# fusiyuan2010/CSC

Measured on AMD Instinct MI355X. Metric: encode MB/s (10^6 input bytes / wall-clock) on enwik9 stand-in, -m3 -d64m; stream bit-exact vs reference, higher is better.
Workload: dtype u8/u32 (byte + 32-bit integer work; 12-bit probabilities, 64-bit range-coder low)

## Files before the change

### csc_amd/csrc/csc_kernels_dp4.inc

```

constexpr uint32_t kD4Rec = 256;
constexpr uint32_t kD4CandEnt = kD4Rec * 4;
constexpr uint32_t kD4RefEnt = 256;
constexpr uint32_t kD4Ent = kD4CandEnt + kD4RefEnt;
constexpr uint32_t kD4LA = 48;
constexpr uint32_t kD4Waves = 12;
DEV uint32_t d4_role(uint32_t w)
{
    constexpr uint32_t roles[12] = { 0, 6, 7, 1, 8, 5, 4, 2, 8, 8, 9, 3 };
    return w < 12 ? roles[w] : 8u;
}
constexpr uint32_t kD4Requested = 0xFFFFFFFFu;
#ifndef D4_IDLE_MUL
#define D4_IDLE_MUL 1
#endif
constexpr int kD4IdleSleep = 4 * D4_IDLE_MUL;
constexpr uint32_t kD4RefreshAt = 32;
constexpr uint32_t kD4MaxGood = 16;
constexpr uint32_t kD6Ring = 128;
constexpr uint32_t kD6MRing = 64;
constexpr uint32_t kD4MultiMax = 768;

struct Dp4X {
    uint32_t sb_seq, sb_ack, quit, abort;
    uint32_t sb0, pos0, size, gen;
    uint32_t m_pos;
    uint32_t m_ids[2];
    uint32_t ins_head;
    uint32_t cmp_next, cmp_pause, cmp_idle[3], cmp_cur[3];
    uint32_t ev_seq, ev_s, ev_len, ev_ack;
    uint32_t ref_head;
    uint32_t rq_head, rq_tail;
    uint32_t lit_req, lit_from, lit_done;
    uint32_t rid[4];
    uint32_t io_w0, io_gen, io_state0, io_lp_int, io_lit_seq, io_rq_head, io_wnd_lo, io_wnd_hi, io_wnd_size, io_vld, io_good, io_plit_lo, io_plit_hi;
    alignas(16) uint32_t o_kind, o_end, o_a0l, o_a0code, o_a0eid, o_a0slot, o_fin_i0, o_fin_i1, o_lp_int, o_lit_seq, o_rq_head, o_err;
#ifdef CSCMI_TIMERS
    uint32_t stat[8];
    uint32_t wtm[52];
#endif
    uint32_t rq[16][2];
    raw_vec4 cand[kD4Rec];
    uint8_t hflag[kD4Rec];
    uint32_t rec_tag[kD4Rec], rec_hsum[kD4Rec], rec_a0d[kD4Rec], rec_len[kD4Rec][16];
    uint32_t rec_m32[kD4Rec][16];
    raw_vec4 ent[kD4Ent];
    uint32_t fwd[kD4Ent];
    alignas(512) uint16_t litp[4][kD4Rec];
    alignas(16) uint16_t tab[64][32];
    alignas(256) raw_vec4 lab[16];
    alignas(512) uint32_t tent[2][16][8];
    alignas(256) raw_vec4 ver[16];
    uint32_t lab_seq, win_seq;
    alignas(16) uint32_t dump[8];
    alignas(8) uint32_t e_prog[2]; uint32_t e_stop[2];
#ifdef CSCMI_TIMERS
    uint32_t dbgp[64], dbgq[64][8], dbgl[32];
    uint32_t dbg;
    uint32_t tr_win, tr_lo, tr_hi;
#endif
    uint32_t lenp_new[32];
    uint32_t lt_pub, lt_done;
    uint32_t lt_rec[kD6Ring];
    uint32_t mt_pub, mt_done;
    uint32_t mt_rec[kD6MRing][2];
    uint32_t hS[2], h_reset, hand[20];
};
struct EncLds4 { EncLds base; Dp4X x; CoderQ q; };
__shared__ EncLds4 g_lds4;

DEV uint32_t d4_tag(uint32_t gen, uint32_t p) { return ((gen << 13) | p) + 1u; }
DEV Dp4X *d4x(Sc &c) { return reinterpret_cast<Dp4X *>(c.X); }

DEV uint32_t d4_eq4(uint32_t x)
{
    const uint32_t z = ~(((x & 0x7F7F7F7Fu) + 0x7F7F7F7Fu) | x) & 0x80808080u;
    return (((z >> 7) * 0x01020408u) >> 24) & 0xFu;
}
DEV uint32_t d4_eq8(uint64_t x) { return d4_eq4((uint32_t)x) | (d4_eq4((uint32_t)(x >> 32)) << 4); }

DEV bool d4_spin(Sc &c, Dp4X *X, uint32_t &spins, uint32_t site)
{
    __builtin_amdgcn_s_sleep(1);
    if ((++spins & 1023u) == 0 && (spins > (kDpSpinLimit << 2) || lds_vload(&X->abort))) {
        if (!lds_vload(&X->abort)) lds_vstore(&X->abort, 0x40000000u | (site << 16) | (c.wv << 24) | (spins & 0xFFFFu));
        c.error = lds_vload(&X->abort);
        return false;
    }
    return true;
}
template <int LANE> DEV uint32_t d4_wrlane(uint32_t old, uint32_t val)
{
// ... 1745 lines not shown
    if (!d6_tree_record(c, X, 0u | (len << 1), dist, d6_len_slots(len) + sbits + ndir + (extra_bits ? 4u : 0u), q)) return false;
    c.state = (c.state * 4 + 1) & 0x3F;
    c.st_match++;
    return true;
}
DEV bool d6_rep_match(Sc &c, Dp4X *X, uint32_t rep_idx, uint32_t len, D6Cur &q)
{
    const uint32_t s3 = c.state * 3, k = c.lane;
    const uint32_t idx = k < 3 ? P_STATE + s3 + k : P_REPDIST + s3 - 1u + (k == 3 ? 1u : 2u | (rep_idx >> 1));
    const uint32_t bit = k < 3 ? (0x5u >> k) & 1u : (rep_idx >> ((4u - k) & 1u)) & 1u;
    d6_flags(c, 5, idx, bit);
    if (!d6_tree_record(c, X, 1u | (len << 1), 0u, d6_len_slots(len), q)) return false;
    c.state = (c.state * 4 + 3) & 0x3F;
    c.st_match++;
    return true;
}
DEV void d6_rep0len1(Sc &c)
{
    d6_flags(c, 3, P_STATE + c.state * 3 + c.lane, c.lane == 0 ? 1u : 0u);
    c.ctx = 0;
    c.state = (c.state * 4 + 2) & 0x3F;
    c.st_match++;
}
DEV bool d6_encode_nonlit(Sc &c, Dp4X *X, uint32_t ulen, uint32_t udist, D6Cur &q)
{
    EncLds *L = c.L;
    if (udist <= 4) {
        if (ulen == 1 && udist == 1) d6_rep0len1(c);
        else {
            if (!d6_rep_match(c, X, udist - 1, ulen - 2, q)) return false;
            uint32_t d = UNI(L->rep[udist - 1]);
            for (uint32_t k = udist - 1; k > 0; k--) L->rep[k] = UNI(L->rep[k - 1]);
            L->rep[0] = d;
        }
    } else {
        if (!d6_match(c, X, udist - 5, ulen - 2, q)) return false;
        uint32_t r0 = UNI(L->rep[0]), r1 = UNI(L->rep[1]), r2 = UNI(L->rep[2]);
        L->rep[3] = r2; L->rep[2] = r1; L->rep[1] = r0; L->rep[0] = udist - 4;
    }
    return true;
}
DEV uint32_t d6_chunk_shape(uint32_t nd, uint32_t ql, bool on)
{
    const uint32_t len = ql & 0xFFFFu;
    const uint32_t kind = nd == 0 ? 0u : nd > 4 ? 1u : (nd == 1 && len == 1) ? 2u : 3u;
    const uint32_t l2 = len - 2u, dist = nd - 5u;
    const uint32_t sbits = l2 == 0 ? 3u : l2 <= 2 ? 4u : 5u;
    const uint32_t slot = dist_slot(dist), extra_bits = slot > 2 ? slot - 2 : 0;
    const uint32_t ndir = extra_bits > 4 ? (extra_bits - 4 > 16 ? 2u : 1u) : 0u;
    const uint32_t nf = kind == 0 ? 1u : kind == 1 ? 2u : kind == 2 ? 3u : 5u;
    const uint32_t tree = kind == 0 ? 8u : kind == 2 ? 0u : d6_len_slots(l2) + (kind == 1 ? sbits + ndir + (extra_bits ? 4u : 0u) : 0u);
    return on ? kind | (nf << 2) | ((nf + tree) << 8) : 0u;
}
DEV void d6_chunk_flag(bool act, uint32_t idx, uint32_t bit, uint32_t qslot, uint64_t same)
{
    const uint64_t am = __ballot(act);
    if (am == 0) return;
    const uint32_t lane = threadIdx.x & 63u;
    same &= am;
    const uint64_t below = same & ((1ull << lane) - 1ull), above = (same >> lane) >> 1;
    const uint32_t rank = (uint32_t)__builtin_popcountll(below);
    const uint32_t prev = below ? 63u - (uint32_t)__builtin_clzll(below) : lane;
    uint32_t pold = 0;
    if (act) pold = g_lds4.base.P[idx];
    uint32_t pnew = p_update(bit, pold);
    for (uint32_t d = 1; __ballot(act && rank >= d) != 0; d++) {
        const uint32_t v = (uint32_t)__builtin_amdgcn_ds_bpermute((int)(prev * 4u), (int)pnew);
        if (act && rank == d) { pold = v; pnew = p_update(bit, pold); }
    }
    if (act && above == 0) g_lds4.base.P[idx] = pnew;
    if (act) g_lds4.q.e[qslot & (kCoderQ - 1)] = 0x80000000u | (bit << 12) | pold;
}
__device__ __noinline__ uint32_t d6_chunk_lanes(uint32_t nd, uint32_t ql, uint32_t shape, uint32_t qpos, uint32_t n_, uint32_t state0_, uint32_t ctx0_, uint32_t lt_head_, uint32_t mt_head_)
{
    Dp4X *X = &g_lds4.x;
    const uint32_t lane = threadIdx.x & 63u;
    const uint32_t n = UNI(n_), state0 = UNI(state0_), ctx0 = UNI(ctx0_), lt_head = UNI(lt_head_), mt_head = UNI(mt_head_);
    const bool on = lane < n;
    const uint32_t kind = shape & 3u, nf = (shape >> 2) & 7u;
    const uint32_t len = ql & 0xFFFFu, last = ql >> 16;
    const uint64_t b0 = __ballot(on && (kind & 1u)), b1 = __ballot(on && (kind & 2u));
    const uint64_t h0 = (b0 << 3) | ((state0 & 1u) << 2) | (((state0 >> 2) & 1u) << 1) | ((state0 >> 4) & 1u);
    const uint64_t h1 = (b1 << 3) | (((state0 >> 1) & 1u) << 2) | (((state0 >> 3) & 1u) << 1) | ((state0 >> 5) & 1u);
    const uint32_t a = (uint32_t)(lane >= 3 ? b0 >> (lane - 3u) : h0 >> lane) & 7u, b = (uint32_t)(lane >= 3 ? b1 >> (lane - 3u) : h1 >> lane) & 7u;
    const uint32_t state = ((a >> 2) & 1u) | (((b >> 2) & 1u) << 1) | (((a >> 1) & 1u) << 2) | (((b >> 1) & 1u) << 3) | ((a & 1u) << 4) | ((b & 1u) << 5);
    const uint32_t before = (uint32_t)__shfl_up((int)last, 1);
    const uint32_t ctx = lane == 0 ? ctx0 : before;
    const bool is_lit = on && kind == 0, has_tree = on && (kind & 1u);
    const uint64_t lm = __ballot(is_lit), tm = __ballot(has_tree);
    if (is_lit) {
        const uint32_t r = __builtin_amdgcn_mbcnt_hi((uint32_t)(lm >> 32), __builtin_amdgcn_mbcnt_lo((uint32_t)lm, 0u));
        *(lds_vu32 *)&X->lt_rec[(lt_head + r) & (kD6Ring - 1)] = ctx | (last << 8) | (qpos << 16);
    }
    if (lm) lds_vstore(&X->lt_pub, lt_head + (uint32_t)__builtin_popcountll(lm));
    if (has_tree) {
        const uint32_t r = __builtin_amdgcn_mbcnt_hi((uint32_t)(tm >> 32), __builtin_amdgcn_mbcnt_lo((uint32_t)tm, 0u));
        *(lds_vu32 *)&X->mt_rec[(mt_head + r) & (kD6MRing - 1)][0] = (kind == 3 ? 1u : 0u) | ((len - 2u) << 1) | ((qpos + nf) << 16);
        *(lds_vu32 *)&X->mt_rec[(mt_head + r) & (kD6MRing - 1)][1] = kind == 1 ? nd - 5u : 0u;
    }
    if (tm) lds_vstore(&X->mt_pub, mt_head + (uint32_t)__builtin_popcountll(tm));
    uint64_t same = 0;
    for (uint64_t rem = __ballot(on); rem;) {
        const uint32_t sv = rdlane(state, (uint32_t)__builtin_ctzll(rem));
        const uint64_t mm = __ballot(on && state == sv);
        same = state == sv ? mm : same;
        rem &= ~mm;
    }
    const uint32_t s3 = state * 3u, rep_hi = ((nd - 1u) >> 1) & 1u;
    const bool is_rep = on && kind == 3;
    d6_chunk_flag(on, P_STATE + s3, kind != 0 ? 1u : 0u, qpos, same);
    d6_chunk_flag(on && kind != 0, P_STATE + s3 + 1u, kind == 1 ? 1u : 0u, qpos + 1u, same);
    d6_chunk_flag(on && kind >= 2, P_STATE + s3 + 2u, kind == 3 ? 1u : 0u, qpos + 2u, same);
    d6_chunk_flag(is_rep, P_REPDIST + s3, rep_hi, qpos + 3u, same);
    const uint64_t hi = __ballot(is_rep && rep_hi);
    d6_chunk_flag(is_rep, P_REPDIST + s3 + 1u + rep_hi, (nd - 1u) & 1u, qpos + 4u, same & (rep_hi ? hi : ~hi));
    return rdlane(((state * 4u + kind) & 0x3Fu) | (last << 8), n - 1u);
}
struct D6Rec {
    uint32_t len;
    uint32_t k0[3], nb[3], x[3], base[3];
    uint32_t n, n_head;
    uint32_t ndir, dir0, dir1;
};
DEV D6Rec d6_rec(uint32_t w0, uint32_t dist)
{
    D6Rec r;
    const uint32_t len = (w0 >> 1) & 0xFFu;
    r.len = len;
    r.k0[0] = len < 8 ? 1u : 2u; r.nb[0] = len < 16 ? 3u : 7u; r.x[0] = len < 8 ? len : len < 16 ? len - 8u : len - 16u;
    r.base[0] = len < 8 ? (uint32_t)P_LEN_X1 : len < 16 ? (uint32_t)P_LEN_X2 : (uint32_t)P_LEN_X3;
    uint32_t n = r.k0[0] + r.nb[0];
    const bool match = (w0 & 1u) == 0;
    const uint32_t sbits = len == 0 ? 3u : len <= 2 ? 4u : 5u;
    const uint32_t pdist_pos = len == 0 ? 0u : len <= 2 ? 16u * (len - 1u) + 8u : 32u * (umin(len, 6u) - 3u) + 8u + 16u * 2u;
    const uint32_t slot = dist_slot(dist), extra_bits = match && slot > 2 ? slot - 2u : 0u;
    r.k0[1] = n; r.nb[1] = match ? sbits : 0u; r.x[1] = slot; r.base[1] = P_DIST + pdist_pos;
    n += r.nb[1];
    r.n_head = n;
    const uint32_t extra_len = dist - (1u << (extra_bits & 31u)) - 1u;
    r.k0[2] = n; r.nb[2] = extra_bits ? 4u : 0u; r.x[2] = __brev(extra_len & 0x0Fu) >> 28; r.base[2] = P_DIST_EXTRA + (extra_bits - 1u) * 16u;
    n += r.nb[2];
    r.n = n;
    const uint32_t v = extra_len >> 4, l = extra_bits - 4u;
    r.ndir = extra_bits > 4 ? (l > 16 ? 2u : 1u) : 0u;
    r.dir0 = l <= 16 ? (l << 16) | (v & 0xFFFFu) : ((l - 16u) << 16) | ((v >> 16) & 0xFFFFu);
    r.dir1 = (16u << 16) | (v & 0xFFFFu);
    return r;
}
DEV void d6_rec_cell(const D6Rec &r, uint32_t k, uint32_t &idx, uint32_t &bit)
{
    idx = P_LEN_SLOT; bit = r.len >= 8 ? 1u : 0u;
    if (k == 1 && r.len >= 8) { idx = P_LEN_SLOT + 1; bit = r.len >= 16 ? 1u : 0u; }
#pragma unroll
    for (uint32_t s = 0; s < 3; s++) {
        const uint32_t l = k - r.k0[s];
        if (l < r.nb[s]) { idx = r.base[s] + ((1u << l) | (r.x[s] >> ((r.nb[s] - l) & 31u))); bit = (r.x[s] >> ((r.nb[s] - 1u - l) & 31u)) & 1u; }
    }
}
DEV uint32_t d6_rec_lane(const D6Rec &r, uint32_t idx)
{
    uint32_t k = 0xFFu;
    if (idx == P_LEN_SLOT) k = 0;
    if (idx == P_LEN_SLOT + 1 && r.len >= 8) k = 1;
#pragma unroll
    for (uint32_t s = 0; s < 3; s++) {
        const uint32_t node = idx - r.base[s];
        const uint32_t l = 31u - (uint32_t)__builtin_clz(node | 1u);
        if (node >= 1u && node < (1u << r.nb[s]) && node == ((1u << l) | (r.x[s] >> ((r.nb[s] - l) & 31u)))) k = r.k0[s] + l;
// ... 95 lines not shown
            prev_a = (i >= j && o == cell_a) ? j : prev_a;
            const uint32_t o2 = (uint32_t)__builtin_amdgcn_ds_bpermute((int)((lane + 8u * j) * 4u), (int)cell_a);
            later_a = later_a || (i + j < 8u && o2 == cell_a);
        }
        uint32_t from_a = 0;
        if (n_b) {
#pragma unroll
            for (uint32_t j = 7; j >= 1; j--) {
                const uint32_t o = (uint32_t)__builtin_amdgcn_ds_bpermute((int)((lane - 8u * j) * 4u), (int)cell_b);
                prev_b = (i >= j && o == cell_b) ? j : prev_b;
                const uint32_t o2 = (uint32_t)__builtin_amdgcn_ds_bpermute((int)((lane + 8u * j) * 4u), (int)cell_b);
                later_b = later_b || (i + j < 8u && o2 == cell_b);
            }
#pragma unroll
            for (uint32_t j = 0; j < 8; j++) {
                const uint32_t r = (i + j) & 7u;
                const uint32_t oa = (uint32_t)__builtin_amdgcn_ds_bpermute((int)((lane + 8u * j) * 4u), (int)cell_a);
                from_a = (oa == cell_b && r + 1u > from_a) ? r + 1u : from_a;
                const uint32_t ob = (uint32_t)__builtin_amdgcn_ds_bpermute((int)((lane + 8u * j) * 4u), (int)cell_b);
                later_a = later_a || ob == cell_a;
            }
        }
        uint32_t pnew_a = p_update(bit_a, pold_a);
        const uint64_t cm_a = __ballot(prev_a != 0);
        if (__builtin_expect(cm_a != 0, 0)) {
            for (uint32_t r = 1; r < n_a; r++) {
                if (((cm_a >> (8u * r)) & 0xFFull) == 0) continue;
                const uint32_t v = (uint32_t)__builtin_amdgcn_ds_bpermute((int)((lane - 8u * prev_a) * 4u), (int)pnew_a);
                if (i == r && prev_a != 0) { pold_a = v; pnew_a = p_update(bit_a, pold_a); }
            }
        }
        if (n_b) {
            if (__ballot(from_a != 0)) {
                const uint32_t v = (uint32_t)__builtin_amdgcn_ds_bpermute((int)(((from_a - 1u) * 8u + k) * 4u), (int)pnew_a);
                pold_b = from_a ? v : pold_b;
            }
            uint32_t pnew_b = p_update(bit_b, pold_b);
            const uint64_t cm_b = __ballot(prev_b != 0);
            if (__builtin_expect(cm_b != 0, 0)) {
                for (uint32_t r = 1; r < n_b; r++) {
                    if (((cm_b >> (8u * r)) & 0xFFull) == 0) continue;
                    const uint32_t v = (uint32_t)__builtin_amdgcn_ds_bpermute((int)((lane - 8u * prev_b) * 4u), (int)pnew_b);
                    if (i == r && prev_b != 0) { pold_b = v; pnew_b = p_update(bit_b, pold_b); }
                }
            }
            if (act_b && !later_b) c.p_lit[cell_b] = pnew_b;
            if (act_b) g_lds4.q.e[((rec_b >> 16) + 1u + k) & (kCoderQ - 1)] = 0x80000000u | (bit_b << 12) | pold_b;
        }
        if (act_a && !later_a) c.p_lit[cell_a] = pnew_a;
        if (act_a) g_lds4.q.e[((rec_a >> 16) + 1u + k) & (kCoderQ - 1)] = 0x80000000u | (bit_a << 12) | pold_a;
        dp_fence();
        done += nlit;
        lds_vstore(&X->lt_done, done);
        pub = lds_vload(&X->lt_pub);
    }
  }
}

DEV void lz_compress_advanced_dp4(Sc &c, uint32_t size)
{
    EncLds *L = c.L;
    Dp4X *X = d4x(c);
    const uint32_t lane = c.lane;
    const uint32_t sb0 = c.wnd_curpos, pos0 = c.pos;
    uint32_t rq_head = lds_vload(&X->rq_head);
    uint32_t ev_seq = lds_vload(&X->ev_seq);
    bool ev_pending = false;
    {
        lds_vstore(&X->sb0, sb0); lds_vstore(&X->pos0, pos0); lds_vstore(&X->size, size);
        lds_vstore(&X->m_pos, 0);
        {
            const uint64_t wa = (uint64_t)(uintptr_t)c.wnd;
            X->io_wnd_lo = (uint32_t)wa; X->io_wnd_hi = (uint32_t)(wa >> 32); X->io_wnd_size = c.wnd_size; X->io_vld = c.vld_rge; X->io_good = c.lz_good_len;
            const uint64_t pa = (uint64_t)(uintptr_t)c.p_lit;
            X->io_plit_lo = (uint32_t)pa; X->io_plit_hi = (uint32_t)(pa >> 32);
        }
        dp_fence();
        const uint32_t seq = lds_vload(&X->sb_seq) + 1;
        lds_vstore(&X->sb_seq, seq);
        uint32_t spins = 0;
        while (lds_vload(&X->sb_ack) != seq) if (!d4_spin(c, X, spins, 5)) return;
        lds_fence();
        uint32_t id0 = 0;
        if (lane == 0) id0 = atomicAdd(&X->ref_head, 4u);
        id0 = UNI(id0);
        if (lane < 4) {
            const uint32_t nid = kD4CandEnt + ((id0 + lane) & (kD4RefEnt - 1));
            raw_vec4 en;
            en.x = L->rep[lane]; en.y = sb0 - 64u; en.z = 0; en.w = 0;
            X->ent[nid] = en;
            X->fwd[nid] = 0;
            X->rid[lane] = nid;
        }
        lds_fence();
        if (!d4_rebase_reps(c, X, sb0, rq_head, true)) return;
    }
    uint32_t gen = lds_vload(&X->gen);
    uint32_t lit_seq = lds_vload(&X->lit_req);
    D6Cur tq;
    tq.lt_head = lds_vload(&X->lt_pub); tq.lt_seen = lds_vload(&X->lt_done); tq.mt_head = lds_vload(&X->mt_pub); tq.mt_seen = lds_vload(&X->mt_done);

    for (uint32_t i = 0; i < size;) {
        if (lds_vload(&X->abort)) { c.error = lds_vload(&X->abort); return; }
        TM_DECL;
        const uint32_t w0 = i;
        lds_vstore(&X->m_pos, i);
        if (ev_pending) {
            uint32_t spins = 0;
            while (lds_vload(&X->ev_ack) != ev_seq) if (!d4_spin(c, X, spins, 6)) return;
            lds_fence();
            gen = lds_vload(&X->gen);
            ev_pending = false;
        }
        TM_ADD(c, 0);
        {
            const uint32_t rs = w0 & (kD4Rec - 1);
            const uint32_t tg = *(lds_vu32 *)&X->rec_tag[rs], hs = *(lds_vu32 *)&X->rec_hsum[rs];
            const uint32_t rid_l = *(lds_vu32 *)&X->rid[lane & 3u];
            const raw_vec4 en = *(lds_vvec4 *)&X->ent[rid_l];
            const uint32_t wpos = sb0 + w0, off = wpos - en.y;
            const uint32_t mlow = (uint32_t)((((uint64_t)en.w << 32) | en.z) >> (off & 63u));
            const uint32_t bad = (off >> 6) | ((((off & 63u) + 1u) >> 6) & mlow) | ((umin(en.x - en.y - 1u, 0x7FFFFFFFu) - off) >> 31) | (((mlow & 3u) + 1u) >> 2);
            if (UNI(tg) == d4_tag(gen, w0) && (UNI(hs) & 0xFFu) == 0 && __ballot(bad != 0) == 0 && w0 + 1u < size && !D5FLAG(30)) {
                if (!d6_room(c, X, 16u, tq)) return;
                if (!d6_literal(c, X, stage_byte(c, sb0 + w0), tq)) return;
                TM_ADD(c, 4);
                c.st_find++;
                i++;
                continue;
            }
        }
        if (!d6_join(c, X, tq, true)) return;
        TM_ADD(c, 5);
        if (__builtin_expect(c.error != 0, 0)) { if (!lds_vload(&X->abort)) lds_vstore(&X->abort, c.error); return; }
        X->io_w0 = w0; X->io_gen = gen; X->io_state0 = c.state; X->io_lp_int = c.lp_rebuild_int; X->io_lit_seq = lit_seq; X->io_rq_head = rq_head;
        lds_fence();
#ifdef CSCMI_TIMERS
        if (D5DBG(32u) && c.lane < 32) X->dbgl[c.lane] = L->len_price[c.lane];
#endif
#ifdef CSCMI_TIMERS
        const bool d5_here = (lds_vload(&X->dbg) >> 8) == 0 || D5DBG(64u) || pos0 + w0 < (lds_vload(&X->dbg) >> 8) * 16u;
#else
        const bool d5_here = true;
#endif
#ifdef CSCMI_TIMERS
        if (kD5Split && !D5DBG(16u) && d5_here) d5_spine();
        else d4_window();
#else
        (void)d5_here;
        d5_spine();
#endif
#ifdef CSCMI_TIMERS
        if (D5DBG(128u) && pos0 + w0 + 1024u >= (lds_vload(&X->dbg) >> 8) * 16u) { for (int q = 0; q < 100; q++) __builtin_amdgcn_s_sleep(127); }
#endif
#ifdef CSCMI_TIMERS
        if (D5DBG(32u) && lds_vload(&X->o_end) < 150u && c.S->stats.trace[62][0] == 0
            && (!D5DBG(64u) || (pos0 + w0 < (lds_vload(&X->dbg) >> 8) * 16u && pos0 + w0 + 16u >= (lds_vload(&X->dbg) >> 8) * 16u))) {
            auto sig = [&]() -> uint32_t {
                uint32_t h = lds_vload(&X->o_kind) * 0x9E3779B1u + lds_vload(&X->o_end);
                h = h * 0x85EBCA6Bu + lds_vload(&X->o_a0l); h = h * 0x85EBCA6Bu + lds_vload(&X->o_a0code); h = h * 0x85EBCA6Bu + lds_vload(&X->o_lp_int);
                if (lds_vload(&X->o_kind) == DP_EXIT_MATCH) { h = h * 0x85EBCA6Bu + lds_vload(&X->o_a0slot); if (lds_vload(&X->o_a0code) > 4) h = h * 0x85EBCA6Bu + UNI(X->ent[lds_vload(&X->o_a0eid)].x); }
                { const uint32_t f0 = lds_vload(&X->o_fin_i0), f1 = lds_vload(&X->o_fin_i1);
                  h = h * 31u + UNI(X->ent[f0 & 0xFFFFu].x); h = h * 31u + UNI(X->ent[f0 >> 16].x); h = h * 31u + UNI(X->ent[f1 & 0xFFFFu].x); h = h * 31u + UNI(X->ent[f1 >> 16].x); }
                for (uint32_t t = lds_vload(&X->o_end); t;) {
                    const uint32_t b = UNI(L->fin2[t * 2u + 1u] & 0xFFFFu), d = UNI(L->fin2[t * 2u]);
                    h = (h ^ (t * 31u + d)) * 0x01000193u;
                    t = b;
                }
                return h;
            };
            auto sig2 = [&]() -> uint32_t {
                uint32_t h = 0;
                for (uint32_t q = 0; q < 32; q++) h = h * 31u + UNI(L->len_price[q]);
                return h;
            };
            auto snap = [&](unsigned long long *T) {
                uint32_t hf = 0, he = 0;
                for (uint32_t q = c.lane; q < kD4Ent; q += 64) { hf += X->fwd[q] * (q * 2u + 1u); const raw_vec4 e = X->ent[q]; he += (e.x * 3u + e.y * 5u + e.z * 7u + e.w * 11u) * (q * 2u + 1u); }
                for (int o = 32; o; o >>= 1) { hf += __shfl_xor(hf, o); he += __shfl_xor(he, o); }
                if (c.lane == 0) {
                    T[0] = hf; T[1] = he; T[2] = lds_vload(&X->ref_head); T[3] = lds_vload(&X->rq_head) | ((unsigned long long)lds_vload(&X->rq_tail) << 32);
                    T[4] = lds_vload(&X->lit_req) | ((unsigned long long)lds_vload(&X->lit_done) << 32); T[5] = lds_vload(&X->m_pos);
                    T[6] = lds_vload(&X->m_ids[0]) | ((unsigned long long)lds_vload(&X->m_ids[1]) << 32); T[7] = lds_vload(&X->gen) | ((unsigned long long)lds_vload(&X->ins_head) << 32);
                    T[8] = lds_vload(&X->o_fin_i0) | ((unsigned long long)lds_vload(&X->o_fin_i1) << 32); T[9] = lds_vload(&X->o_kind) | ((unsigned long long)lds_vload(&X->o_end) << 32);
                    T[10] = lds_vload(&X->o_a0eid) | ((unsigned long long)lds_vload(&X->o_a0slot) << 32); T[11] = pos0 + w0;
// ... 8 lines not shown
            X->io_lit_seq = lds_vload(&X->o_lit_seq);
            if (c.lane < 32) L->len_price[c.lane] = X->dbgl[c.lane];
            lds_fence();
            d4_window();
            const uint32_t s4 = sig();
            if (D5DBG(64u)) snap(c.S->stats.trace[59]);
            const uint32_t t4 = sig2();
            if (t4 != t5 && c.S->stats.trace[62][0] == 0 && c.lane == 0) { unsigned long long *T = c.S->stats.trace[62]; T[0] = 2; T[1] = pos0 + w0; T[2] = t5; T[3] = t4; T[4] = lds_vload(&X->io_lp_int); T[5] = lds_vload(&X->o_lp_int); T[6] = lds_vload(&X->o_end); }
            if (s4 != s5 && c.S->stats.trace[62][0] == 0) {
                if (c.lane < 60) { c.S->stats.trace[c.lane][2] = L->fin2[c.lane * 2u]; c.S->stats.trace[c.lane][3] = L->fin2[c.lane * 2u + 1u] & 0xFFFFu; c.S->stats.trace[c.lane][4] = X->dbgp[c.lane]; for (int q = 0; q < 7; q++) c.S->stats.trace[c.lane][5 + q] = X->dbgq[c.lane][q == 6 ? 7 : q]; c.S->stats.trace[c.lane][11] |= (unsigned long long)X->dbgq[c.lane][6] << 32; }
                if (c.lane == 0) {
                    unsigned long long *T = c.S->stats.trace[62];
                    T[0] = 1; T[1] = pos0 + w0; T[2] = k5; T[3] = e5; T[4] = l5; T[5] = a5; T[6] = c5;
                    T[7] = lds_vload(&X->o_kind); T[8] = lds_vload(&X->o_end); T[9] = lds_vload(&X->o_lp_int); T[10] = lds_vload(&X->o_a0l); T[11] = lds_vload(&X->io_lp_int);
                    unsigned long long *U = c.S->stats.trace[63];
                    const uint32_t q0 = lds_vload(&X->o_fin_i0), q1 = lds_vload(&X->o_fin_i1);
                    U[1] = r5a; U[2] = r5b; U[3] = r5c; U[4] = r5d; U[5] = sl5; U[6] = X->ent[q0 & 0xFFFFu].x; U[7] = X->ent[q0 >> 16].x; U[8] = X->ent[q1 & 0xFFFFu].x; U[9] = X->ent[q1 >> 16].x; U[10] = lds_vload(&X->o_a0slot);
                }
            }
        }
#endif
        const raw_vec4 o0 = *(lds_vvec4 *)&X->o_kind, o1 = *(lds_vvec4 *)&X->o_a0eid, o2 = *(lds_vvec4 *)&X->o_lp_int;
        const uint32_t kind = UNI(o0.x), end = UNI(o0.y);
        uint32_t a0l = UNI(o0.z);
        const uint32_t a0code = UNI(o0.w), a0eid = UNI(o1.x), a0slot = UNI(o1.y);
        const uint32_t fin_i0 = UNI(o1.z), fin_i1 = UNI(o1.w);
        c.lp_rebuild_int = UNI(o2.x); lit_seq = UNI(o2.y); rq_head = UNI(o2.z);
        c.st_find += end + (kind == DP_EXIT_LIMIT ? 0u : 1u);
        TM_ADD(c, 1);
#ifdef CSCMI_TIMERS
        if (D5FLAG(29) && c.S->stats.trace[62][0] == 0) {
            const uint32_t thr = lds_vload(&X->tr_win) & 0x1FFFFFFFu;
            if (sb0 + w0 <= thr && thr < sb0 + w0 + end + 1u + (kind == DP_EXIT_MATCH ? a0l : 0u)) {
                if (c.lane < 60) { c.S->stats.trace[c.lane][0] = L->fin2[c.lane * 2u]; c.S->stats.trace[c.lane][1] = L->fin2[c.lane * 2u + 1u]; }
                if (c.lane == 0) {
                    unsigned long long *T = c.S->stats.trace[62];
                    T[0] = 7; T[1] = sb0 + w0; T[2] = kind; T[3] = end; T[4] = a0l; T[5] = a0code; T[6] = a0slot; T[7] = X->ent[fin_i0 & 0xFFFFu].x; T[8] = X->ent[fin_i0 >> 16].x;
                    T[9] = X->ent[fin_i1 & 0xFFFFu].x; T[10] = X->ent[fin_i1 >> 16].x; T[11] = c.state;
                    unsigned long long *U = c.S->stats.trace[63];
                    U[1] = L->rep[0]; U[2] = L->rep[1]; U[3] = L->rep[2]; U[4] = L->rep[3]; U[5] = fin_i0; U[6] = fin_i1; U[7] = X->rid[0] | ((unsigned long long)X->rid[1] << 32); U[8] = X->rid[2] | ((unsigned long long)X->rid[3] << 32);
                    U[9] = X->fwd[X->rid[0]]; U[10] = X->ent[X->rid[0]].y; U[11] = lds_vload(&X->rq_head) | ((unsigned long long)lds_vload(&X->rq_tail) << 32);
                }
            }
        }
#endif
        if (kind == DP_ABORT || UNI(o2.w)) { c.error = lds_vload(&X->abort) | 0x08000000u; return; }
        if (kind == DP_SEEN_EXIT) {
            if (lane < 4) X->rid[lane] = lane == 0 ? fin_i0 & 0xFFFFu : lane == 1 ? fin_i0 >> 16 : lane == 2 ? fin_i1 & 0xFFFFu : fin_i1 >> 16;
            wave_fence();
            if (!d6_room(c, X, 16u, tq)) return;
            if (!d6_literal(c, X, stage_byte(c, sb0 + w0), tq)) return;
            i++;
            TM_ADD(c, 7);
            continue;
        }
        c.wnd_curpos = sb0 + w0 + end;
        if (kind == DP_EXIT_MATCH) {
            if (a0l >= 64u && a0slot >= 4) {
                const uint32_t mp = sb0 + w0 + end, d = a0code - 4u;
                const bool fwd = a0slot == 4 ? (mp > d) : (mp >= d);
                const uint32_t cp = fwd ? mp - d : mp + c.wnd_size - d;
                a0l = wave_prefix_from(c, mp, cp, 64u, umin(size - (w0 + end), c.wnd_size - cp));
            }
            lds_vstore(&X->ev_s, w0 + end); lds_vstore(&X->ev_len, a0l);
            lds_fence();
            ev_seq++;
            lds_vstore(&X->ev_seq, ev_seq);
            ev_pending = true;
        }
        {
            const uint32_t id = lane == 0 ? fin_i0 & 0xFFFFu : lane == 1 ? fin_i0 >> 16 : lane == 2 ? fin_i1 & 0xFFFFu : fin_i1 >> 16;
            if (lane < 4) { X->rid[lane] = id; L->rep[lane] = X->ent[id].x; }
        }
        wave_fence();
        if (kind == DP_EXIT_MATCH) {
            const uint32_t i0 = lds_vload(&X->rid[0]), i1 = lds_vload(&X->rid[1]), i2 = lds_vload(&X->rid[2]), i3 = lds_vload(&X->rid[3]);
            if (a0code > 4) { X->rid[0] = a0eid; X->rid[1] = i0; X->rid[2] = i1; X->rid[3] = i2; }
            else if (a0code == 2) { X->rid[0] = i1; X->rid[1] = i0; }
            else if (a0code == 3) { X->rid[0] = i2; X->rid[1] = i0; X->rid[2] = i1; }
            else if (a0code == 4) { X->rid[0] = i3; X->rid[1] = i0; X->rid[2] = i1; X->rid[3] = i2; }
            wave_fence();
            if (a0l > kD4RefreshAt && w0 + end + a0l < size && !d4_rebase_reps(c, X, sb0 + w0 + end + a0l, rq_head, false)) return;
        }
        TM_ADD(c, 6);
        uint32_t pm_lo = 0, pm_hi = 0;
        for (uint32_t t = end; t;) {
            const uint32_t ch = t >> 6;
            const uint32_t Bv = L->fin2[(ch * 64u + lane) * 2u + 1u] & 0xFFFFu;
            uint64_t m = 0;
            do { m |= 1ull << (t & 63u); t = rdlane(Bv, t & 63u); } while (t && (t >> 6) == ch);
            pm_lo = d4_m0_wrlane(pm_lo, UNI((uint32_t)m), UNI(ch));
            pm_hi = d4_m0_wrlane(pm_hi, UNI((uint32_t)(m >> 32)), UNI(ch));
        }
        TM_ADD(c, 2);
        for (uint32_t ch = 0; ch <= (end >> 6); ch++) {
            const uint64_t m = ((uint64_t)rdlane(pm_hi, ch) << 32) | rdlane(pm_lo, ch);
            if (m == 0) continue;
            const uint32_t n = (uint32_t)__builtin_popcountll(m);
            const uint32_t q = ch * 64u + lane;
            const uint32_t back = L->fin2[q * 2u + 1u] & 0xFFFFu, ndv = L->fin2[q * 2u];
            const uint32_t sidx = w0 + q + 15u;
            const uint32_t lastb = (L->stage[sidx >> 2] >> ((sidx & 3u) * 8u)) & 0xFFu;
            const bool isp = (m >> lane) & 1ull;
            const uint32_t rank = __builtin_amdgcn_mbcnt_hi((uint32_t)(m >> 32), __builtin_amdgcn_mbcnt_lo((uint32_t)m, 0u));
            const uint32_t tgt = (isp ? rank : n + (lane - rank)) * 4u;
            const uint32_t d_nd = (uint32_t)__builtin_amdgcn_ds_permute((int)tgt, (int)ndv);
// ... 3 lines not shown
#pragma unroll
            for (uint32_t b = 0; b < 5; b++) {
                const uint64_t pm = __ballot((shape >> (8u + b)) & 1u);
                qoff += __builtin_amdgcn_mbcnt_hi((uint32_t)(pm >> 32), __builtin_amdgcn_mbcnt_lo((uint32_t)pm, 0u)) << b;
                need += (uint32_t)__builtin_popcountll(pm) << b;
            }
            const uint32_t nl = (uint32_t)__builtin_popcountll(__ballot(lane < n && (shape & 3u) == 0)), nm = (uint32_t)__builtin_popcountll(__ballot(shape & 1u));
            if (!d6_room(c, X, need, tq)) return;
            if (tq.lt_head + nl - tq.lt_seen > kD6Ring - 8u) tq.lt_seen = lds_vload(&X->lt_done);
            if (tq.mt_head + nm - tq.mt_seen > kD6MRing) tq.mt_seen = lds_vload(&X->mt_done);
            const bool at_once = c.q_room >= need && tq.lt_head + nl - tq.lt_seen <= kD6Ring - 8u && tq.mt_head + nm - tq.mt_seen <= kD6MRing;
            TM_ADD(c, 3);
            if (at_once) {
                const uint32_t sc = UNI(d6_chunk_lanes(d_nd, d_ql, shape, c.q_head + qoff, n, c.state, c.ctx, tq.lt_head, tq.mt_head));
                c.state = sc & 0x3Fu; c.ctx = sc >> 8;
                c.q_head += need; c.q_room -= need;
                tq.lt_head += nl; tq.mt_head += nm;
                c.st_lit += nl; c.st_match += n - nl;
                continue;
            }
            for (uint32_t r = 0; r < n; r++) {
                const uint32_t nd = rdlane(d_nd, r), ql = rdlane(d_ql, r);
                const uint32_t len = ql & 0xFFFFu, last = ql >> 16;
                if (nd == 0) {
                    if (!d6_literal(c, X, last, tq)) return;
                    TMF_ADD(c, 4);
                } else if (nd <= 4) {
                    if (len == 1 && nd == 1) d6_rep0len1(c);
                    else if (!d6_rep_match(c, X, nd - 1, len - 2, tq)) return;
                    c.ctx = last;
                    TMF_ADD(c, 7);
                } else {
                    if (!d6_match(c, X, nd - 5, len - 2, tq)) return;
                    c.ctx = last;
                    TMF_ADD(c, 7);
                }
            }
        }
        i += end;
        if (!d6_room(c, X, 256u, tq)) return;
        if (kind == DP_EXIT_LIT) {
            if (!d6_literal(c, X, stage_byte(c, sb0 + i), tq)) return;
            i++;
        } else if (kind == DP_EXIT_MATCH) {
            if (a0l >= 145u) {
                if (!d6_join(c, X, tq)) return;
                lz_encode_nonlit(c, a0l, a0code);
            } else if (!d6_encode_nonlit(c, X, a0l, a0code, tq)) return;
            c.st_slide += a0l - 1;
            i += a0l;
            c.ctx = stage_byte(c, sb0 + i - 1);
        }
        TM_ADD(c, 7);
    }
    if (!d6_join(c, X, tq)) return;
    {
        lds_vstore(&X->m_pos, size);
        uint32_t spins = 0;
        if (ev_pending) { while (lds_vload(&X->ev_ack) != ev_seq) if (!d4_spin(c, X, spins, 9)) return; }
        while (lds_vload(&X->ins_head) < size) if (!d4_spin(c, X, spins, 10)) return;
        if (!d4_quiesce(c, X)) return;
        dp_fence();
    }
    c.pos = pos0 + size;
    c.wnd_curpos = sb0 + size;
}

__device__ __noinline__ void d4_master_nl()
{
    Dp4X *X = &g_lds4.x;
    Sc c;
    const uint64_t sp = ((uint64_t)lds_vload(&X->hS[1]) << 32) | lds_vload(&X->hS[0]);
    const GLOBAL_AS EncState *G = (const GLOBAL_AS EncState *)(uintptr_t)sp;
    c.S = (EncState *)(uintptr_t)sp; c.L = &g_lds4.base; c.X = X; c.Q = &g_lds4.q;
    c.lane = threadIdx.x & 63;
    c.wnd = (gu8 *)uni_gptr(G->wnd); c.wnd_size = UNI(G->wnd_size); c.vld_rge = UNI(G->vld_rge);
    c.ht2 = nullptr; c.ht3 = nullptr; c.ht6 = nullptr; c.bt_head = nullptr; c.bt_nodes = nullptr;
    c.p_lit = (gu32 *)uni_gptr(G->p_lit); c.p_delta = nullptr; c.mfbuf = nullptr; c.swapbuf = nullptr;
    c.ht6_off = 0; c.bth_off = 0; c.fast_ht = true;
    c.gm6 = c.gm2 = c.gm3 = c.gmb = 0; c.gslot = 31; c.pr_off = 0; c.pr_rmask = 0; c.pr_pol = 0;
    c.ht_bits = 0; c.ht_width = 0; c.ht_low = 1; c.ht_cyc = 0; c.bt_bits = 0; c.bt_size = 0; c.bt_cyc = 0;
    c.lz_good_len = UNI(G->lz_good_len); c.lz_bt_cyc = 0; c.lz_ht_cyc = 0; c.good_len = c.lz_good_len;
    c.bt_pos = 0;
    c.rc_low = 0; c.rc_range = 0; c.rc_cache = 0; c.rc_cachesize = 0; c.rc_size = 0; c.bc_size = 0; c.bc_curbits = 0; c.bc_curval = 0; c.bsize = 0;
    c.rc_buf = nullptr; c.bc_buf = nullptr; c.arena = nullptr; c.arena_used = 0; c.arena_cap = 0; c.error = 0;
    c.cand_len_v = 0; c.cand_dist_v = 0;
    c.wv = 0; c.dp_seq = 0; c.dp_idle = 0; c.dp_seq_seen = 0;
    c.st_find = c.st_slide = c.st_bt = c.st_lit = c.st_match = 0;
    c.pipe_ok = 0; c.piped = 0; c.tok_headl = 0; c.tok_tail_seen = 0; c.pipe_seq = 0; c.pair_ok = 1;
#ifdef CSCMI_TIMERS
    for (int k = 0; k < 16; k++) c.tm[k] = 0;
#endif
    c.wnd_curpos = lds_vload(&X->hand[0]); c.stage_base = lds_vload(&X->hand[1]); c.stage_end = lds_vload(&X->hand[2]);
    c.pos = lds_vload(&X->hand[3]); c.state = lds_vload(&X->hand[5]); c.ctx = lds_vload(&X->hand[6]);
    c.lp_rebuild_int = lds_vload(&X->hand[7]); c.q_head = lds_vload(&X->hand[8]); c.q_room = lds_vload(&X->hand[9]);
    const uint32_t size = lds_vload(&X->hand[10]);
    lz_compress_advanced_dp4(c, size);
    if (c.lane == 0) {
        X->hand[0] = c.wnd_curpos; X->hand[3] = c.pos; X->hand[5] = c.state; X->hand[6] = c.ctx;
        X->hand[7] = c.lp_rebuild_int; X->hand[8] = c.q_head; X->hand[9] = c.q_room; X->hand[11] = c.error;
        X->hand[12] = c.st_find; X->hand[13] = c.st_slide; X->hand[14] = c.st_bt; X->hand[15] = c.st_lit; X->hand[16] = c.st_match;
#ifdef CSCMI_TIMERS
        for (int q = 0; q < 8; q++) atomicAdd(&c.S->stats.tm[q], c.tm[q]);
#endif
    }
    lds_fence();
// ... 66 lines not shown
                }
                return;
            }
            __builtin_amdgcn_s_sleep(2);
        }
        lds_acquire();
#ifdef CSCMI_TIMERS
        const uint64_t tc0 = __builtin_readcyclecounter();
        const uint32_t tail0 = tail;
#endif
        while (tail != pub) {
            const uint32_t n = umin(pub - tail, 64u);
            const uint32_t ev = Q->e[(tail + c.lane) & (kCoderQ - 1)];
            for (uint32_t j = 0; j < n; j++) {
                const uint32_t e = rdlane(ev, j);
                if (e & 0x80000000u) rc_code(c, (e >> 12) & 1u, e & 0xFFFu);
                else if (e & 0x40000000u) enc_direct16(c, e & 0xFFFFu, (e >> 16) & 0x1Fu);
                else coder_flush(c);
            }
            tail += n;
            lds_vstore(&Q->tail, tail);
        }
#ifdef CSCMI_TIMERS
        if (c.lane == 0) { atomicAdd(&X->wtm[43], (uint32_t)(__builtin_readcyclecounter() - tc0) >> 4); atomicAdd(&X->wtm[44], tail - tail0); atomicAdd(&X->wtm[45], 1u); }
#endif
    }
}

DEV void d4_worker(Sc &c)
{
    c.wv = d4_role(c.wv);
    if (c.wv == 8) return;
    if (c.wv == 1) d4_inserter(c);
    else if (c.wv == 9) d6_trees(c);
    else if (c.wv == 4) d4_service(c);
    else if (c.wv == 5) d4_coder(c);
    else if (c.wv >= 6) d5_edges(c, c.wv - 6u);
    else d4_compare(c, c.wv == 2 ? 0u : 1u);
}
DEV void d4_quit(Sc &c)
{
    Dp4X *X = d4x(c);
    if (c.Q) {
        q_publish(c);
        uint32_t spins = 0;
        while (lds_vload(&c.Q->tail) != c.q_head) if (!d4_spin(c, X, spins, 11)) break;
    }
    dp_fence();
    lds_vstore(&X->quit, 1);
    if (!c.error && lds_vload(&X->abort)) c.error = lds_vload(&X->abort);
#ifdef CSCMI_TIMERS
    for (int q = 2; q < 8; q++) c.tm[8 + q] += lds_vload(&X->stat[q]);
    if (g_lds4.x.dbgl[31] && c.S->stats.trace[61][0] == 0 && c.lane < 4 && g_lds4.x.dbgq[c.lane][2]) { unsigned long long *T = c.S->stats.trace[60]; T[12 * 0 + c.lane * 3 + 0] = g_lds4.x.dbgq[c.lane][0] + ((unsigned long long)g_lds4.x.dbgq[c.lane][4] << 32); T[c.lane * 3 + 1] = g_lds4.x.dbgq[c.lane][1] + ((unsigned long long)g_lds4.x.dbgq[c.lane][3] << 32); T[c.lane * 3 + 2] = g_lds4.x.dbgq[c.lane][2]; c.S->stats.trace[61][0] = 1; }
    if (c.lane == 0) for (int q = 0; q < 52; q++) atomicAdd((unsigned long long *)&c.S->stats.trace[q / 12][q % 12], (unsigned long long)lds_vload(&X->wtm[q]));
#endif
}
```

Measured before the change: 3.058.

## Replace serial per-flag bpermute chains with bitmask replay of probability updates

The chunk-lane flag coder drops the per-flag serial ds_bpermute chain and the iterative state-grouping loop. The same-state lane mask is now built directly from the state-history ballots. Each lane loads its probability cell once and replays the adaptive updates of the earlier same-context lanes from ballot bitmasks, and writes are steered to a dump slot instead of branching. Extra timer-only instrumentation (join timing, replay rounds) is added under CSCMI_TIMERS. The replay loop still runs as many rounds as the longest predecessor chain, and it depends on the dump cell and q.pad existing.

```diff
diff --git a/csc_amd/csrc/csc_kernels_dp4.inc b/csc_amd/csrc/csc_kernels_dp4.inc
--- a/csc_amd/csrc/csc_kernels_dp4.inc
+++ b/csc_amd/csrc/csc_kernels_dp4.inc
@@ -37,7 +37,7 @@
     alignas(16) uint32_t o_kind, o_end, o_a0l, o_a0code, o_a0eid, o_a0slot, o_fin_i0, o_fin_i1, o_lp_int, o_lit_seq, o_rq_head, o_err;
 #ifdef CSCMI_TIMERS
     uint32_t stat[8];
-    uint32_t wtm[52];
+    uint32_t wtm[68];
 #endif
     uint32_t rq[16][2];
     raw_vec4 cand[kD4Rec];
@@ -1889,24 +1889,25 @@
     const uint32_t tree = kind == 0 ? 8u : kind == 2 ? 0u : d6_len_slots(l2) + (kind == 1 ? sbits + ndir + (extra_bits ? 4u : 0u) : 0u);
     return on ? kind | (nf << 2) | ((nf + tree) << 8) : 0u;
 }
-DEV void d6_chunk_flag(bool act, uint32_t idx, uint32_t bit, uint32_t qslot, uint64_t same)
-{
-    const uint64_t am = __ballot(act);
-    if (am == 0) return;
-    const uint32_t lane = threadIdx.x & 63u;
-    same &= am;
-    const uint64_t below = same & ((1ull << lane) - 1ull), above = (same >> lane) >> 1;
-    const uint32_t rank = (uint32_t)__builtin_popcountll(below);
-    const uint32_t prev = below ? 63u - (uint32_t)__builtin_clzll(below) : lane;
-    uint32_t pold = 0;
-    if (act) pold = g_lds4.base.P[idx];
-    uint32_t pnew = p_update(bit, pold);
-    for (uint32_t d = 1; __ballot(act && rank >= d) != 0; d++) {
-        const uint32_t v = (uint32_t)__builtin_amdgcn_ds_bpermute((int)(prev * 4u), (int)pnew);
-        if (act && rank == d) { pold = v; pnew = p_update(bit, pold); }
-    }
-    if (act && above == 0) g_lds4.base.P[idx] = pnew;
-    if (act) g_lds4.q.e[qslot & (kCoderQ - 1)] = 0x80000000u | (bit << 12) | pold;
+DEV uint32_t d6_chunk_replay(uint32_t p, uint64_t preds, uint64_t bits, uint32_t plane)
+{
+    (void)plane;
+#ifdef CSCMI_TIMERS
+    uint32_t rounds = 0;
+#endif
+    while (__ballot(preds != 0) != 0) {
+        const uint32_t t = (uint32_t)__builtin_ctzll(preds | (1ull << 63));
+        const uint32_t pu = p + (uint32_t)((int32_t)((((uint32_t)(bits >> t) & 1u) ? 0xFFFu : 31u) - p) >> 5);
+        p = preds ? pu : p;
+        preds &= preds - 1ull;
+#ifdef CSCMI_TIMERS
+        rounds++;
+#endif
+    }
+#ifdef CSCMI_TIMERS
+    if ((threadIdx.x & 63u) == 0 && rounds) atomicAdd(&g_lds4.x.wtm[61 + plane], rounds);
+#endif
+    return p;
 }
 __device__ __noinline__ uint32_t d6_chunk_lanes(uint32_t nd, uint32_t ql, uint32_t shape, uint32_t qpos, uint32_t n_, uint32_t state0_, uint32_t ctx0_, uint32_t lt_head_, uint32_t mt_head_)
 {
@@ -1936,21 +1937,46 @@
         *(lds_vu32 *)&X->mt_rec[(mt_head + r) & (kD6MRing - 1)][1] = kind == 1 ? nd - 5u : 0u;
     }
     if (tm) lds_vstore(&X->mt_pub, mt_head + (uint32_t)__builtin_popcountll(tm));
-    uint64_t same = 0;
-    for (uint64_t rem = __ballot(on); rem;) {
-        const uint32_t sv = rdlane(state, (uint32_t)__builtin_ctzll(rem));
-        const uint64_t mm = __ballot(on && state == sv);
-        same = state == sv ? mm : same;
-        rem &= ~mm;
-    }
+#ifdef CSCMI_TIMERS
+    if (lane == 0) atomicAdd(&X->wtm[66], 1u);
+#endif
     const uint32_t s3 = state * 3u, rep_hi = ((nd - 1u) >> 1) & 1u;
     const bool is_rep = on && kind == 3;
-    d6_chunk_flag(on, P_STATE + s3, kind != 0 ? 1u : 0u, qpos, same);
-    d6_chunk_flag(on && kind != 0, P_STATE + s3 + 1u, kind == 1 ? 1u : 0u, qpos + 1u, same);
-    d6_chunk_flag(on && kind >= 2, P_STATE + s3 + 2u, kind == 3 ? 1u : 0u, qpos + 2u, same);
-    d6_chunk_flag(is_rep, P_REPDIST + s3, rep_hi, qpos + 3u, same);
-    const uint64_t hi = __ballot(is_rep && rep_hi);
-    d6_chunk_flag(is_rep, P_REPDIST + s3 + 1u + rep_hi, (nd - 1u) & 1u, qpos + 4u, same & (rep_hi ? hi : ~hi));
+    const uint64_t in0 = state0 & 1u, in1 = (state0 >> 1) & 1u;
+    const uint64_t B0 = (b0 << 1) | in0, B1 = (b1 << 1) | in1;
+    const uint64_t B2 = (b0 << 2) | (in0 << 1) | ((state0 >> 2) & 1u), B3 = (b1 << 2) | (in1 << 1) | ((state0 >> 3) & 1u);
+    const uint64_t onm = __ballot(on);
+    uint64_t same = onm;
+    same &= (state & 1u) ? B0 : ~B0;   same &= (state & 2u) ? B1 : ~B1;
+    same &= (state & 4u) ? B2 : ~B2;   same &= (state & 8u) ? B3 : ~B3;
+    same &= (state & 16u) ? h0 : ~h0;  same &= (state & 32u) ? h1 : ~h1;
+    static_assert(P_REPDIST >= P_STATE + 64 * 3 && P_DIST >= P_REPDIST + 64 * 3, "the flag planes' cells: two ranges of 3 a state");
+    const uint64_t below_all = same & ((1ull << lane) - 1ull), above_all = same & ~((2ull << lane) - 1ull);
+    const uint64_t am1 = onm & ~lm, am2 = __ballot(on && kind >= 2), am3 = __ballot(is_rep), hi = __ballot(is_rep && rep_hi);
+    const uint64_t sm4 = am3 & (rep_hi ? hi : ~hi);
+    const bool act1 = on && kind != 0, act2 = on && kind >= 2;
+    const uint32_t bit0 = kind != 0 ? 1u : 0u, bit1 = kind == 1 ? 1u : 0u, bit2 = kind == 3 ? 1u : 0u, bit4 = (nd - 1u) & 1u;
+    const uint32_t i0 = on ? P_STATE + s3 : kPDumpE, i1 = act1 ? P_STATE + s3 + 1u : kPDumpE, i2 = act2 ? P_STATE + s3 + 2u : kPDumpE;
+    const uint32_t i3 = is_rep ? P_REPDIST + s3 : kPDumpE, i4 = is_rep ? P_REPDIST + s3 + 1u + rep_hi : kPDumpE;
+    uint32_t *const P = g_lds4.base.P;
+    uint32_t p0 = P[i0], p1 = P[i1], p2 = P[i2], p3 = P[i3], p4 = P[i4];
+    const uint64_t bits1 = __ballot(act1 && bit1), bits4 = __ballot(is_rep && bit4);
+    p0 = d6_chunk_replay(p0, on ? below_all : 0ull, am1, 0);
+    p1 = d6_chunk_replay(p1, act1 ? below_all & am1 : 0ull, bits1, 1);
+    p2 = d6_chunk_replay(p2, act2 ? below_all & am2 : 0ull, am3, 2);
+    p3 = d6_chunk_replay(p3, is_rep ? below_all & am3 : 0ull, hi, 3);
+    p4 = d6_chunk_replay(p4, is_rep ? below_all & sm4 : 0ull, bits4, 4);
+    P[above_all == 0 ? i0 : kPDumpE] = p0 + (uint32_t)((int32_t)((bit0 ? 0xFFFu : 31u) - p0) >> 5);
+    P[(above_all & am1) == 0 ? i1 : kPDumpE] = p1 + (uint32_t)((int32_t)((bit1 ? 0xFFFu : 31u) - p1) >> 5);
+    P[(above_all & am2) == 0 ? i2 : kPDumpE] = p2 + (uint32_t)((int32_t)((bit2 ? 0xFFFu : 31u) - p2) >> 5);
+    P[(above_all & am3) == 0 ? i3 : kPDumpE] = p3 + (uint32_t)((int32_t)((rep_hi ? 0xFFFu : 31u) - p3) >> 5);
+    P[(above_all & sm4) == 0 ? i4 : kPDumpE] = p4 + (uint32_t)((int32_t)((bit4 ? 0xFFFu : 31u) - p4) >> 5);
+    lds_vu32 *const spare = (lds_vu32 *)&g_lds4.q.pad;
+    *(on ? (lds_vu32 *)&g_lds4.q.e[qpos & (kCoderQ - 1)] : spare) = 0x80000000u | (bit0 << 12) | p0;
+    *(act1 ? (lds_vu32 *)&g_lds4.q.e[(qpos + 1u) & (kCoderQ - 1)] : spare) = 0x80000000u | (bit1 << 12) | p1;
+    *(act2 ? (lds_vu32 *)&g_lds4.q.e[(qpos + 2u) & (kCoderQ - 1)] : spare) = 0x80000000u | (bit2 << 12) | p2;
+    *(is_rep ? (lds_vu32 *)&g_lds4.q.e[(qpos + 3u) & (kCoderQ - 1)] : spare) = 0x80000000u | (rep_hi << 12) | p3;
+    *(is_rep ? (lds_vu32 *)&g_lds4.q.e[(qpos + 4u) & (kCoderQ - 1)] : spare) = 0x80000000u | (bit4 << 12) | p4;
     return rdlane(((state * 4u + kind) & 0x3Fu) | (last << 8), n - 1u);
 }
 struct D6Rec {
@@ -2152,6 +2178,9 @@
         dp_fence();
         done += nlit;
         lds_vstore(&X->lt_done, done);
+#ifdef CSCMI_TIMERS
+        if (lane == 0) { atomicAdd(&X->wtm[59], 1u); atomicAdd(&X->wtm[60], nlit); }
+#endif
         pub = lds_vload(&X->lt_pub);
     }
   }
@@ -2200,6 +2229,9 @@
     D6Cur tq;
     tq.lt_head = lds_vload(&X->lt_pub); tq.lt_seen = lds_vload(&X->lt_done); tq.mt_head = lds_vload(&X->mt_pub); tq.mt_seen = lds_vload(&X->mt_done);
 
+#ifdef CSCMI_TIMERS
+    uint32_t tj_last = 2;
+#endif
     for (uint32_t i = 0; i < size;) {
         if (lds_vload(&X->abort)) { c.error = lds_vload(&X->abort); return; }
         TM_DECL;
@@ -2225,12 +2257,22 @@
                 if (!d6_room(c, X, 16u, tq)) return;
                 if (!d6_literal(c, X, stage_byte(c, sb0 + w0), tq)) return;
                 TM_ADD(c, 4);
+#ifdef CSCMI_TIMERS
+                tj_last = 2;
+#endif
                 c.st_find++;
                 i++;
                 continue;
             }
         }
+#ifdef CSCMI_TIMERS
+        const uint64_t tj0 = __builtin_readcyclecounter();
+        const uint32_t tj_out = tq.lt_head - lds_vload(&X->lt_done);
+#endif
         if (!d6_join(c, X, tq, true)) return;
+#ifdef CSCMI_TIMERS
+        if (c.lane == 0) { atomicAdd(&X->wtm[52 + tj_last], (uint32_t)(__builtin_readcyclecounter() - tj0) >> 4); atomicAdd(&X->wtm[55 + tj_last], 1u); atomicAdd(&X->wtm[58], tj_out); }
+#endif
         TM_ADD(c, 5);
         if (__builtin_expect(c.error != 0, 0)) { if (!lds_vload(&X->abort)) lds_vstore(&X->abort, c.error); return; }
         X->io_w0 = w0; X->io_gen = gen; X->io_state0 = c.state; X->io_lp_int = c.lp_rebuild_int; X->io_lit_seq = lit_seq; X->io_rq_head = rq_head;
@@ -2345,6 +2387,9 @@
             if (!d6_literal(c, X, stage_byte(c, sb0 + w0), tq)) return;
             i++;
             TM_ADD(c, 7);
+#ifdef CSCMI_TIMERS
+            tj_last = 2;
+#endif
             continue;
         }
         c.wnd_curpos = sb0 + w0 + end;
@@ -2454,6 +2499,9 @@
             c.ctx = stage_byte(c, sb0 + i - 1);
         }
         TM_ADD(c, 7);
+#ifdef CSCMI_TIMERS
+        tj_last = kind == DP_EXIT_LIT ? 0u : 1u;
+#endif
     }
     if (!d6_join(c, X, tq)) return;
     {
@@ -2626,6 +2674,6 @@
 #ifdef CSCMI_TIMERS
     for (int q = 2; q < 8; q++) c.tm[8 + q] += lds_vload(&X->stat[q]);
     if (g_lds4.x.dbgl[31] && c.S->stats.trace[61][0] == 0 && c.lane < 4 && g_lds4.x.dbgq[c.lane][2]) { unsigned long long *T = c.S->stats.trace[60]; T[12 * 0 + c.lane * 3 + 0] = g_lds4.x.dbgq[c.lane][0] + ((unsigned long long)g_lds4.x.dbgq[c.lane][4] << 32); T[c.lane * 3 + 1] = g_lds4.x.dbgq[c.lane][1] + ((unsigned long long)g_lds4.x.dbgq[c.lane][3] << 32); T[c.lane * 3 + 2] = g_lds4.x.dbgq[c.lane][2]; c.S->stats.trace[61][0] = 1; }
-    if (c.lane == 0) for (int q = 0; q < 52; q++) atomicAdd((unsigned long long *)&c.S->stats.trace[q / 12][q % 12], (unsigned long long)lds_vload(&X->wtm[q]));
-#endif
-}
+    if (c.lane == 0) for (int q = 0; q < 68; q++) atomicAdd((unsigned long long *)&c.S->stats.trace[q / 12][q % 12], (unsigned long long)lds_vload(&X->wtm[q]));
+#endif
+}
```

After: 3.079 (median of 6 runs). About the same (+0.7%).
